# espresso3389/MioTTS-llama.cpp

Hardware: AMD Instinct MI355X
Metric: realtime factor (audio s / wall s) + stage ms llm/codec/istft, 1.7B Q4_K_M (higher is better)
Workload: dtype int8-dot (q4_K/q6_K x q8_K) + f32/f16 codec; 1 GPU; MioTTS-1.7B Q4_K_M single utterance, 700 speech tokens -> MioCodec -> iSTFT (28.0 s audio each) per GPU; model=MioTTS-1.7B Q4_K_M, global_batch=1, seq_len=700, parallelism=utterance-sharded x1 (no collective), devices_visible=1

## Files before the change

### miotts-llama.cpp_amd/csrc/hip/llm_attention.h

```cpp
#pragma once
#include "llm_device.h"

namespace mio {
namespace {

__device__ inline float load_resid(const float *x, int lo, int hi) {
    const int lane = threadIdx.x & 63;
    return lo + lane < hi ? x[lo + lane] : 0.0f;
}
__device__ inline float lane_value(float v, int i) {
    return __int_as_float(__builtin_amdgcn_readlane(__float_as_int(v), i));
}

template <int HD, int G, bool DG, bool WQ = false>
__device__ __forceinline__ bool attention_wg(const LlmDims &d, const float *q_norm, const float *k_norm,
                                             const float *bqkv, _Float16 *kc, _Float16 *vc, const LlmBuffers &b,
                                             int ch, int kvh, int pos, int *rdy) {
    constexpr bool kDiag = DG;
    using C = AttCfg<HD>;
    constexpr int PER = HD / 64;
    __shared__ float qs[G][HD];
    __shared__ float knew[HD], vnew[HD];
    using A = AttM<HD>;
    static_assert(C::NT == A::NT, "attention workgroup size");
// ... 61 lines not shown
    attend_chunk_mfma<HD, G>(qh, img, img + A::IMG, t0, pos, d.scale, b.part + head0 + (uint32_t)ch * C::REC, gs,
                             DG ? b.trace : nullptr);
    attn_merge_last<HD, G>(b.part, head0, gs, pos / ATT_CHUNK + 1, b.att_cnt + kvh, b.att + (size_t)kvh * G * HD, -1,
                           {}, 0, rdy, (kDiag && b.tl) ? MIO_TL_SLOT(b) : nullptr);
    return true;
}

template <int NP, int T, int SU, bool DG>
__device__ __forceinline__ void o_consumer(const LlmDims &d, const QMat &wo, const LlmBuffers &b, int ob, int no) {
    constexpr bool kDiag = DG;
    extern __shared__ __attribute__((aligned(16))) char smem[];
    const int K = wo.k;
    const Smem s = carve(smem, K);
    int lo, hi;
    wave_range(wo.rows, lo, hi, ob, no);
    const float xres = load_resid(b.x, lo, hi);
    Frag ga[Cfg<NP, SU>::U], gb[Cfg<NP, SU>::U];
    load_first<T, NP, 1, SU, MIO_SMALL_AUX>(wo, wo, lo, hi, ga, gb);
    if (MIO_TIDX == 0)
        wait_count(b.att_cnt + kRdyOff + kRdyStride * (blockIdx.x & (kRdyShards - 1)), d.n_kv, b.att_cnt + kRdyFlag);
    asm volatile("s_barrier" ::: "memory");
    MIO_TL_MARK(b, 3);
    XRegs<NP> xr;
    load_x<NP, 16>(b.att, nullptr, K, xr);
    x_after_weights(xr);
    MIO_TL_MARK1(b);
    plain_quant(xr, K, akind(T), s, MIO_TL_DIAGSLOT(b));
    MIO_TL_MARK(b, 2);
    stream_rows_lanes<T, NP, 1, SU, MIO_SMALL_AUX>(wo, wo, lo, hi, ga, gb, s.a, [&](int row, float v, float) {
        b.x[row] = v + xres;
    });
}

}
}
```

### miotts-llama.cpp_amd/csrc/hip/llm_device.h

```cpp
#pragma once

#include <cfloat>
#include <climits>
#include <cstdio>
#include <cstdlib>
#include <type_traits>

#include "llm_kernels.h"

#pragma clang fp contract(off)

#ifndef MIO_TIDX
#define MIO_TIDX threadIdx.x
#endif

namespace mio {
namespace {
constexpr bool kDiag = true;
#define MIO_TRACE(bufs, k)                                                                    \
    do {                                                                                      \
        if (kDiag && (bufs).trace && blockIdx.x == 0 && blockIdx.y == 0 && MIO_TIDX == 0) { \
            asm volatile("" ::: "memory");                                                    \
            (bufs).trace[k] = __builtin_readcyclecounter();                                   \
            if ((k) == 0 || (k) == 15) (bufs).trace[16 + (k)] = __builtin_amdgcn_s_memrealtime(); \
// ... 291 lines not shown
    float4 w[XV];
};

template <int XV>
__device__ __forceinline__ void x_after_weights(XRegs<XV> &xr) {
#pragma unroll
    for (int i = 0; i < XV; ++i)
        asm volatile("" : "+v"(xr.v[i].x), "+v"(xr.v[i].y), "+v"(xr.v[i].z), "+v"(xr.v[i].w), "+v"(xr.w[i].x),
                     "+v"(xr.w[i].y), "+v"(xr.w[i].z), "+v"(xr.w[i].w));
}

template <int XV, int XAUX = 0>
__device__ inline void load_x(const float *x, const float *w, int K, XRegs<XV> &xr) {
    const auto rx = __builtin_amdgcn_make_buffer_rsrc(const_cast<float *>(x), 0, x ? K * 4 : 0, 0x00020000);
    const auto rw = __builtin_amdgcn_make_buffer_rsrc(const_cast<float *>(w), 0, w ? K * 4 : 0, 0x00020000);
#pragma unroll
    for (int i = 0; i < XV; ++i) {
        const int e = (MIO_TIDX + i * MT) * 4;
        const u32x4 a = __builtin_amdgcn_raw_buffer_load_b128(rx, e * 4, 0, XAUX);
        const u32x4 c = __builtin_amdgcn_raw_buffer_load_b128(rw, e * 4, 0, 0);
        xr.v[i] = make_float4(__uint_as_float(a.x), __uint_as_float(a.y), __uint_as_float(a.z), __uint_as_float(a.w));
        xr.w[i] = make_float4(__uint_as_float(c.x), __uint_as_float(c.y), __uint_as_float(c.z), __uint_as_float(c.w));
    }
}

__host__ __device__ constexpr int akind(int T) { return T == 30 ? 2 : (T == 8 ? 0 : 1); }

__device__ __forceinline__ uint32_t f32_to_bf16(float f) {
    const uint32_t u = __float_as_uint(f);
    if ((u & 0x7fffffffu) > 0x7f800000u) return (u >> 16) | 64u;
    return (u + (0x7fffu + ((u >> 16) & 1u))) >> 16;
}

template <int XV>
__device__ __forceinline__ void quant_regs(const float4 (&v)[XV], int K, int ak, const ActL &a) {
    const int lane = MIO_TIDX & 63, wave = __builtin_amdgcn_readfirstlane(MIO_TIDX >> 6);
    if (ak == 1) {
        q8k_regs<XV>(v, K, a);
    } else if (ak == 2) {
#pragma unroll
        for (int j = 0; j < XV; ++j) {
            const int e = (MIO_TIDX + j * MT) * 4;
            if (e < K)
                *reinterpret_cast<uint2 *>(a.qs + 2 * e) =
                    make_uint2(f32_to_bf16(v[j].x) | (f32_to_bf16(v[j].y) << 16),
                               f32_to_bf16(v[j].z) | (f32_to_bf16(v[j].w) << 16));
// ... 275 lines not shown
        r.lo = *reinterpret_cast<const int4 *>(a.qs + e);
        r.hi = *reinterpret_cast<const int4 *>(a.qs + e2);
        r.b0 = a.bs[e >> 4];
        r.b1 = a.bs[e2 >> 4];
        r.d = a.d[sbc];
    } else if constexpr (T == 30) {
        auto at = [&](int i) {
            const int e = min(pass * 2048 + 512 * i + 8 * lane, K - 8);
            return *reinterpret_cast<const int4 *>(a.qs + 2 * e);
        };
        r.lo = at(0), r.hi = at(1), r.lo2 = at(2), r.hi2 = at(3);
        r.b0 = r.b1 = 0;
        r.d = 0.0f;
    } else {
        const int nb = K >> 5, b = pass * 64 + lane, bc = b < nb ? b : 0;
        r.lo = *reinterpret_cast<const int4 *>(a.qs + 32 * bc);
        r.hi = *reinterpret_cast<const int4 *>(a.qs + 32 * bc + 16);
        r.b0 = r.b1 = 0;
        r.d = a.d[bc];
    }
    return r;
}

template <int T>
__device__ __forceinline__ float dot_frag(const Frag &f, const ALane &al, int K, int pass) {
    const int lane = MIO_TIDX & 63;
    if constexpr (T == 12 || T == 13) {
        const int jj = (lane & 7) >> 1;
        uint4 h;
        auto bc = [&]<int CTRL>() {
            if constexpr (T == 12) return (uint32_t)dpp_perm<CTRL>((int)f.c);
            else return (uint32_t)dpp_i<CTRL>((int)f.c);
        };
        h.x = bc.template operator()<0x00>();
        h.y = bc.template operator()<0x55>();
        h.z = bc.template operator()<0xAA>();
        h.w = bc.template operator()<0xFF>();
        const uint32_t wlo = jj < 2 ? h.y : (jj == 2 ? h.z : h.w);
        const uint32_t whi = jj < 2 ? h.z : h.w;
        const uint32_t F = __builtin_amdgcn_alignbit(whi, wlo, (24 * jj) & 31);
        const int sc0 = F & 63, m0 = (F >> 6) & 63, sc1 = (F >> 12) & 63, m1 = (F >> 18) & 63;
        auto lo = [&](uint32_t q, uint32_t h) {
            if constexpr (T == 13) return (int)((q & M4) | (((h >> (2 * jj)) & 0x01010101u) << 4));
            else return (int)(q & M4);
        };
        auto hi = [&](uint32_t q, uint32_t h) {
            if constexpr (T == 13) return (int)(((q >> 4) & M4) | (((h >> (2 * jj + 1)) & 0x01010101u) << 4));
            else return (int)((q >> 4) & M4);
        };
        int dlo = 0, dhi = 0;
        dlo = sdot4(lo(f.a.x, f.b.x), al.lo.x, dlo);
        dlo = sdot4(lo(f.a.y, f.b.y), al.lo.y, dlo);
        dlo = sdot4(lo(f.a.z, f.b.z), al.lo.z, dlo);
        dlo = sdot4(lo(f.a.w, f.b.w), al.lo.w, dlo);
        dhi = sdot4(hi(f.a.x, f.b.x), al.hi.x, dhi);
        dhi = sdot4(hi(f.a.y, f.b.y), al.hi.y, dhi);
        dhi = sdot4(hi(f.a.z, f.b.z), al.hi.z, dhi);
        dhi = sdot4(hi(f.a.w, f.b.w), al.hi.w, dhi);
        int isum = __mul24(sc0, dlo) + __mul24(sc1, dhi);
        int imin = __mul24(m0, al.b0) + __mul24(m1, al.b1);
        isum = sum8_i(isum);
        imin = sum8_i(imin);
        const float d = h2f(h.x & 0xFFFF) * al.d;
        const float dmin = h2f(h.x >> 16) * al.d;
        float v = d * (float)isum;
        v = v - dmin * (float)imin;
        return pass * 8 + (lane >> 3) < (K >> 8) ? v : 0.0f;
    } else if constexpr (T == 14) {
        const int shl = 2 * ((lane & 3) >> 1);
        auto lo = [&](uint32_t l, uint32_t h) { return (int)((l & M4) | ((h << (4 - shl)) & 0x30303030u)); };
        auto hi = [&](uint32_t l, uint32_t h) { return (int)(((l >> 4) & M4) | ((h >> shl) & 0x30303030u)); };
        int dlo = 0, dhi = 0;
        dlo = sdot4(lo(f.a.x, f.b.x), al.lo.x, dlo);
        dlo = sdot4(lo(f.a.y, f.b.y), al.lo.y, dlo);
        dlo = sdot4(lo(f.a.z, f.b.z), al.lo.z, dlo);
        dlo = sdot4(lo(f.a.w, f.b.w), al.lo.w, dlo);
        dhi = sdot4(hi(f.a.x, f.b.x), al.hi.x, dhi);
        dhi = sdot4(hi(f.a.y, f.b.y), al.hi.y, dhi);
        dhi = sdot4(hi(f.a.z, f.b.z), al.hi.z, dhi);
        dhi = sdot4(hi(f.a.w, f.b.w), al.hi.w, dhi);
        const int sa = (int)(int8_t)(f.c & 0xFF), sb = (int)(int8_t)(f.c >> 8);
        int isum = __mul24(sa, dlo - 32 * al.b0) + __mul24(sb, dhi - 32 * al.b1);
        isum = sum8_i(isum);
        const float d = h2f(f.e) * al.d;
        const float v = d * (float)isum;
        return pass * 8 + (lane >> 3) < (K >> 8) ? v : 0.0f;
    } else if constexpr (T == 30) {
        typedef __bf16 bf2 __attribute__((ext_vector_type(2)));
        float acc = 0.0f;
        auto dot8 = [&](const uint4 &w, const int4 &x, int i) {
            const bool ok = pass * 2048 + 512 * i + 8 * lane < K;
            const uint4 ww = ok ? w : make_uint4(0, 0, 0, 0);
            const uint4 xx = ok ? make_uint4((uint32_t)x.x, (uint32_t)x.y, (uint32_t)x.z, (uint32_t)x.w)
                                : make_uint4(0, 0, 0, 0);
            acc = __builtin_amdgcn_fdot2_f32_bf16(__builtin_bit_cast(bf2, ww.x), __builtin_bit_cast(bf2, xx.x), acc, false);
            acc = __builtin_amdgcn_fdot2_f32_bf16(__builtin_bit_cast(bf2, ww.y), __builtin_bit_cast(bf2, xx.y), acc, false);
            acc = __builtin_amdgcn_fdot2_f32_bf16(__builtin_bit_cast(bf2, ww.z), __builtin_bit_cast(bf2, xx.z), acc, false);
            acc = __builtin_amdgcn_fdot2_f32_bf16(__builtin_bit_cast(bf2, ww.w), __builtin_bit_cast(bf2, xx.w), acc, false);
        };
        dot8(f.a, al.lo, 0);
        dot8(f.b, al.hi, 1);
        dot8(f.a2, al.lo2, 2);
        dot8(f.b2, al.hi2, 3);
        return acc;
    } else {
        int s = 0;
        s = sdot4((int)f.a.x, al.lo.x, s);
        s = sdot4((int)f.a.y, al.lo.y, s);
        s = sdot4((int)f.a.z, al.lo.z, s);
        s = sdot4((int)f.a.w, al.lo.w, s);
        s = sdot4((int)f.b.x, al.hi.x, s);
        s = sdot4((int)f.b.y, al.hi.y, s);
        s = sdot4((int)f.b.z, al.hi.z, s);
        s = sdot4((int)f.b.w, al.hi.w, s);
        const float v = (float)s * (h2f(f.e) * al.d);
        return pass * 64 + lane < (K >> 5) ? v : 0.0f;
    }
}

template <int T>
__device__ __forceinline__ float row_total(float acc) {
    if constexpr (T == 8 || T == 30) acc = sum8_f(acc);
    return sum_lanes7(acc);
}

template <int NP, int SU = 0>
struct Cfg {
    static constexpr int U = SU ? SU : (NP == 1 ? 4 : 3);
    static constexpr int NG = SU ? 1 : 2;
    static constexpr bool AREG = NP <= 3;
};

template <int T, int NP, int NM, int SU = 0, int AUX = MIO_WEIGHT_AUX>
__device__ __forceinline__ void load_group(const QMat W0, const QMat W1, int lo, int n, int u0,
                                           Frag (&f)[Cfg<NP, SU>::U], int split = INT_MAX) {
#pragma unroll
    for (int j = 0; j < Cfg<NP, SU>::U; ++j) {
        const int u = __builtin_amdgcn_readfirstlane(max(0, min(u0 + j, n - 1)));
        const int p = u % NP, m = (u / NP) % NM, i = u / (NP * NM);
        if constexpr (NM == 1) {
            const int r = __builtin_amdgcn_readfirstlane(lo + i);
            f[j] = load_frag<T, AUX>(r >= split ? W1 : W0, r >= split ? r - split : r, p);
        } else {
            f[j] = load_frag<T, AUX>(m ? W1 : W0, lo + i, p);
        }
    }
}

// ... 44 lines not shown
                }
            }
        }
    };
    for (int u0 = 0;;) {
        consume(A, u0);
        if (trace && u0 == 0 && blockIdx.x == 0 && MIO_TIDX == 0) trace[3] = __builtin_readcyclecounter();
        if constexpr (Cfg<NP, SU>::NG == 1) break;
        u0 += U;
        if (u0 >= n) break;
        load_group<T, NP, NM, SU, AUX>(W0, W1, lo, n, u0 + U, A, split);
        consume(B, u0);
        u0 += U;
        if (u0 >= n) break;
        load_group<T, NP, NM, SU, AUX>(W0, W1, lo, n, u0 + U, B, split);
    }
}

template <int T, int NP, int NM, int SU = 0, int AUX = MIO_WEIGHT_AUX, class Fin>
__device__ __forceinline__ void stream_rows_lanes(const QMat W0, const QMat W1, int lo, int hi,
                                                  Frag (&A)[Cfg<NP, SU>::U], Frag (&B)[Cfg<NP, SU>::U], const ActL &a,
                                                  Fin &&fin, int split = INT_MAX, unsigned long long *trace = nullptr) {
    const int lane = MIO_TIDX & 63;
    if constexpr (SU != 0 && SU / (NM * NP) == 1) {
        stream_rows<T, NP, NM, SU, AUX>(W0, W1, lo, hi, A, B, a, [&](int row, float v0, float v1) {
            if (lane == 0) fin(row, v0, v1);
        }, split, trace);
        return;
    }
    float p0 = 0.0f, p1 = 0.0f;
    stream_rows<T, NP, NM, SU, AUX>(W0, W1, lo, hi, A, B, a, [&](int row, float v0, float v1) {
        const int k = (row - lo) & 63;
        p0 = lane == k ? v0 : p0;
        if constexpr (NM == 2) p1 = lane == k ? v1 : p1;
        if constexpr (SU == 0) {
            if (k == 63) fin(row - 63 + lane, p0, p1);
        }
    }, split, trace);
    const int rest = SU == 0 ? (hi - lo) & 63 : hi - lo;
    if (lane < rest) fin(hi - rest + lane, p0, p1);
}

template <int T, int NP, int NM, int SU = 0, int AUX = MIO_WEIGHT_AUX>
__device__ __forceinline__ void load_first(const QMat W0, const QMat W1, int lo, int hi, Frag (&A)[Cfg<NP, SU>::U],
                                           Frag (&B)[Cfg<NP, SU>::U], int split = INT_MAX) {
    const int n = (hi - lo) * NM * NP;
// ... 614 lines not shown
```

### miotts-llama.cpp_amd/csrc/hip/llm_kernels.h

```cpp
#pragma once

#include <hip/hip_runtime.h>

#include <cstdint>

namespace mio {

#ifndef MIO_ATT_CHUNK
#define MIO_ATT_CHUNK 64
#endif
constexpr int kAttChunk = MIO_ATT_CHUNK;
constexpr int kTlSlots = 2048;
static_assert(kAttChunk == 32 || kAttChunk == 64 || kAttChunk == 128, "attention chunk");

struct QMat {
    int type;
    int rows, k;
    const uint8_t *p0, *p1, *p2, *p3;
};

inline QMat qmat_rows(const QMat &q, int r0, int n) {
    size_t rb[4] = {0, 0, 0, 0};
    switch (q.type) {
        case 8: rb[0] = (size_t)q.k, rb[1] = (size_t)q.k / 32 * 2; break;
// ... 161 lines not shown
    int g = rows / 8;
    g = g < n_wg ? g : n_wg;
    return g < 2 ? 2 : g;
}
int matvec_grid(const LlmDims &d, int rows);
bool att_o_supported(int hd, int G);
bool layer_att_supported(const LlmDims &d, const LayerW &L);
bool ffn_fused_supported(const LlmDims &d, const LayerW &L);
void launch_layer_att(const LlmDims &d, const LayerW &L, _Float16 *kc, _Float16 *vc, const LlmBuffers &b, bool dg,
                      hipStream_t s);
constexpr int kRdyOff = 64, kRdyShards = 8, kRdyStride = 64;
constexpr int kRdyFlag = kRdyOff + kRdyShards * kRdyStride;
constexpr int kQkvOff = kRdyFlag + 64, kQkvStride = 64, kQkvMax = 64;
constexpr int kFfnOff = kQkvOff + kQkvStride * kQkvMax, kFfnShards = 8, kFfnStride = 64;
constexpr int kFfnRdy = kFfnOff + kFfnShards * kFfnStride;
constexpr int kAttCntInts = kFfnRdy + kFfnShards * kFfnStride;
int pick_np(int K);
size_t matvec_lds(int K);
int max_wave_units(int rows, int grid, int np, int nm);
int pick_su(int units, int np);
void launch_attn_in(const LlmDims &d, const LayerW &L, int il, const QMat &tok_embd, const LlmBuffers &b, bool dg,
                    hipStream_t s);
void launch_debug_matvec(const QMat &W, const QMat *up, const float *x, float *y, int n_wg, hipStream_t s);
size_t debug_act_record_bytes(int K);
void launch_debug_act_quant(int type, const float *x, const float *w, int K, float eps, bool sc1, void *out,
                            hipStream_t s);
size_t debug_act_bytes(int K);
void launch_debug_mmq(const QMat &W, const QMat &up, int mode, const float *x, int nt, char *act, float *y,
                      hipStream_t s);

}
```

### miotts-llama.cpp_amd/csrc/hip/llm_kernels.hip

```cpp
#include "llm_attention.h"

#include <algorithm>
#include <cstdlib>

#pragma clang fp contract(off)

namespace mio {
namespace {



template <int NP, int T, int SU, bool DG>
__global__ __launch_bounds__(MT) void k_attn_out(LlmDims d, QMat wo, LlmBuffers b) {
    constexpr bool kDiag = DG;
    extern __shared__ __attribute__((aligned(16))) char smem[];
    MIO_TRACE(b, 0);
    MIO_TL_BEGIN(b);
    const int K = wo.k;
    const Smem s = carve(smem, K);
    int lo, hi;
    wave_range(d, wo.rows, lo, hi);
    const uint32_t dn = done_issue(b);
    XRegs<NP> xr;
    load_x(b.att, nullptr, K, xr);
    const float xres = load_resid(b.x, lo, hi);
    Frag ga[Cfg<NP, SU>::U], gb[Cfg<NP, SU>::U];
    load_first<T, NP, 1, SU, MIO_SMALL_AUX>(wo, wo, lo, hi, ga, gb);
    x_after_weights(xr);
    if (done_now(dn)) return;
    MIO_TRACE(b, 1);
    MIO_TL_MARK1(b);
    plain_quant(xr, K, akind(T), s, MIO_TL_DIAGSLOT(b));
    MIO_TRACE(b, 2);
    MIO_TL_MARK(b, 2);
    stream_rows_lanes<T, NP, 1, SU, MIO_SMALL_AUX>(wo, wo, lo, hi, ga, gb, s.a, [&](int row, float v, float) {
        b.x[row] = v + xres;
    });
    MIO_TL_END(b);
    MIO_TRACE(b, 15);
}

template <int NP, int T, int SU, bool DG>
__global__ __launch_bounds__(MT) void k_conv_out(LlmDims d, QMat wo, const float *conv_w, float *ring, LlmBuffers b) {
    constexpr bool kDiag = DG;
    extern __shared__ __attribute__((aligned(16))) char smem[];
    MIO_TRACE(b, 0);
    MIO_TL_BEGIN(b);
    const int K = wo.k;
    const Smem s = carve(smem, K);
    const uint32_t dn = done_issue(b);
    const int pos = cur_pos(b.st, d);
// ... 58 lines not shown
    MIO_TRACE(b, 1);
    MIO_TL_MARK1(b);
    rmsnorm_quant(xr, K, d.eps, akind(T), s, MIO_TL_DIAGSLOT(b));
    MIO_TRACE(b, 2);
    MIO_TL_MARK(b, 2);
    stream_rows_lanes<T, NP, 2, SU>(gate, up, lo, hi, ga, gb, s.a, [&](int row, float g, float u) {
        b.h[row] = silu_f(g) * u;
    }, INT_MAX, DG ? b.trace : nullptr);
    if (adv && blockIdx.x == 0 && MIO_TIDX == 0) advance_state(b.st, d);
    MIO_TL_END(b);
    MIO_TRACE(b, 15);
}

template <int NP, int T, int SU, bool DG>
__global__ __launch_bounds__(MT) void k_ffn_down(LlmDims d, QMat down, LlmBuffers b) {
    constexpr bool kDiag = DG;
    extern __shared__ __attribute__((aligned(16))) char smem[];
    MIO_TRACE(b, 0);
    MIO_TL_BEGIN(b);
    const int K = down.k;
    const Smem s = carve(smem, K);
    const uint32_t dn = done_issue(b);
    XRegs<NP> xr;
    load_x(b.h, nullptr, K, xr);
    int lo, hi;
    wave_range(d, down.rows, lo, hi);
    const float xres = load_resid(b.x, lo, hi);
    Frag ga[Cfg<NP, SU>::U], gb[Cfg<NP, SU>::U];
    load_first<T, NP, 1, SU>(down, down, lo, hi, ga, gb);
    x_after_weights(xr);
    if (done_now(dn)) return;
    MIO_TRACE(b, 1);
    MIO_TL_MARK1(b);
    plain_quant(xr, K, akind(T), s, MIO_TL_DIAGSLOT(b));
    MIO_TRACE(b, 2);
    MIO_TL_MARK(b, 2);
    stream_rows_lanes<T, NP, 1, SU>(down, down, lo, hi, ga, gb, s.a, [&](int row, float v, float) {
        b.x[row] = v + xres;
    }, INT_MAX, DG ? b.trace : nullptr);
    MIO_TL_END(b);
    MIO_TRACE(b, 15);
}

template <int NP, int T, int SU, int NPD, int TD, int SUD, bool DG>
__global__ __launch_bounds__(MT) void k_ffn(LlmDims d, const float *norm_w, QMat gate, QMat up, QMat down,
                                            LlmBuffers b, int adv, int GI) {
    constexpr bool kDiag = DG;
    extern __shared__ __attribute__((aligned(16))) char smem[];
    MIO_TRACE(b, 0);
    MIO_TL_BEGIN(b);
    const uint32_t dn = done_issue(b);
    if ((int)blockIdx.x < GI) {
        const int K = d.n_embd;
// ... 31 lines not shown
                last = __hip_atomic_fetch_add((__attribute__((address_space(1))) int *)(b.att_cnt + kFfnOff + kFfnStride * sh),
                                              1, __ATOMIC_RELAXED, __HIP_MEMORY_SCOPE_AGENT) == n_sh - 1;
            }
            if (__builtin_amdgcn_readfirstlane(last) && MIO_TIDX < kFfnShards)
                __hip_atomic_fetch_add((__attribute__((address_space(1))) int *)(b.att_cnt + kFfnRdy + kFfnStride * MIO_TIDX),
                                       1, __ATOMIC_RELAXED, __HIP_MEMORY_SCOPE_AGENT);
        }
    } else {
        const int K = down.k;
        const Smem s = carve(smem, K);
        const int GD = (int)gridDim.x - GI, ob = (int)blockIdx.x - GI;
        int lo, hi;
        wave_range(down.rows, lo, hi, ob, GD);
        const float xres = load_resid(b.x, lo, hi);
        Frag ga[Cfg<NPD, SUD>::U], gb[Cfg<NPD, SUD>::U];
        load_first<TD, NPD, 1, SUD>(down, down, lo, hi, ga, gb);
        if (done_now(dn)) return;
        if (MIO_TIDX == 0)
            wait_count(b.att_cnt + kFfnRdy + kFfnStride * (blockIdx.x & (kFfnShards - 1)), min(GI, kFfnShards),
                       b.att_cnt + kRdyFlag);
        asm volatile("s_barrier" ::: "memory");
        MIO_TL_MARK(b, 3);
        XRegs<NPD> xr;
        load_x<NPD, 16>(b.h, nullptr, K, xr);
        x_after_weights(xr);
        MIO_TL_MARK1(b);
        plain_quant(xr, K, akind(TD), s, MIO_TL_DIAGSLOT(b));
        MIO_TL_MARK(b, 2);
        stream_rows_lanes<TD, NPD, 1, SUD>(down, down, lo, hi, ga, gb, s.a, [&](int row, float v, float) {
            b.x[row] = v + xres;
        });
    }
    MIO_TL_END(b);
    MIO_TRACE(b, 15);
}

#define MIO_FFN_SHAPES(X) \
    X(1, 12, 6, 3, 12, 3)  \
    X(1, 12, 6, 3, 14, 3)  \
    X(1, 13, 6, 3, 13, 3)  \
    X(1, 13, 6, 3, 14, 3)  \
    X(1, 14, 6, 3, 14, 3)  \
    X(1, 30, 6, 3, 30, 3)  \
    X(1, 8, 2, 1, 8, 1)    \
    X(1, 8, 2, 1, 14, 1)   \
    X(1, 8, 0, 6, 8, 0)    \
    X(1, 14, 0, 6, 14, 0)

// ... 362 lines not shown
```

### miotts-llama.cpp_amd/csrc/testlib/debug_capi.cpp

```cpp
#include <cstring>
#include <vector>

#include "common.h"
#include "gguf.h"
#include "llm.h"
#include "llm_kernels.h"
#include "mio_hip_test.h"
#include "quant.h"

namespace {
int debug_matvec(mio_hip_device *d, uint32_t type, const void *gguf_rows, const void *gguf_up, int rows, int k,
                 const float *x, float *y) {
    MIO_REQUIRE(d && gguf_rows && x && y && rows > 0 && k > 0, MIO_ERR_INVALID, "debug_matvec: bad args");
    MIO_REQUIRE(type == mio::GGML_Q8_0 || type == mio::GGML_Q4_K || type == mio::GGML_Q5_K ||
                    type == mio::GGML_Q6_K || type == mio::GGML_BF16 || (!gguf_up && mio::repacks_to_q8_0(type)),
                MIO_ERR_UNSUPPORTED, "debug_matvec: type %u", type);
    const bool k32 = type == mio::GGML_Q8_0 || type == mio::GGML_BF16 || mio::repacks_to_q8_0(type);
    MIO_REQUIRE(k % (k32 ? 32 : 256) == 0, MIO_ERR_INVALID, "debug_matvec: k %d", k);
    int rc = mio::bind(d);
    if (rc) return rc;
    std::vector<uint8_t> q80;
    if (mio::repacks_to_q8_0(type)) {
        q80.resize((size_t)rows * (k / 32) * sizeof(mio::BlockQ8_0));
        mio::repack_to_q8_0(type, gguf_rows, rows, k, q80.data());
        gguf_rows = q80.data();
        type = mio::GGML_Q8_0;
    }
    const mio::SplitLayout L = mio::split_layout(type, rows, k);
    const int nm = gguf_up ? 2 : 1;
    std::vector<uint8_t> host(L.bytes * nm);
    mio::to_split(type, gguf_rows, rows, k, host.data());
    if (gguf_up) mio::to_split(type, gguf_up, rows, k, host.data() + L.bytes);
    uint8_t *dw = nullptr;
    float *dx = nullptr, *dy = nullptr;
    MIO_HIP_CHECK(hipMalloc(&dw, L.bytes * nm));
    MIO_HIP_CHECK(hipMalloc(&dx, (size_t)k * 4));
    MIO_HIP_CHECK(hipMalloc(&dy, (size_t)rows * 4));
    hipMemcpy(dw, host.data(), L.bytes * nm, hipMemcpyHostToDevice);
    hipMemcpy(dx, x, (size_t)k * 4, hipMemcpyHostToDevice);
    auto qm = [&](uint8_t *base) {
        return mio::QMat{(int)type, rows, k, base + L.off[0], base + L.off[1], base + L.off[2], base + L.off[3]};
    };
    const mio::QMat q = qm(dw), up = qm(dw + (gguf_up ? L.bytes : 0));
    mio::launch_debug_matvec(q, gguf_up ? &up : nullptr, dx, dy, d->n_cu > 0 ? d->n_cu : 256, d->stream);
    hipError_t e = hipStreamSynchronize(d->stream);
    if (e == hipSuccess) e = hipMemcpy(y, dy, (size_t)rows * 4, hipMemcpyDeviceToHost);
    hipFree(dw), hipFree(dx), hipFree(dy);
    MIO_HIP_CHECK(e);
    return MIO_OK;
}
}

extern "C" int mio_hip_debug_matvec(mio_hip_device *d, uint32_t type, const void *gguf_rows, int rows, int k,
                                    const float *x, float *y) {
    return debug_matvec(d, type, gguf_rows, nullptr, rows, k, x, y);
}

extern "C" int mio_hip_debug_matvec_swiglu(mio_hip_device *d, uint32_t type, const void *gguf_gate,
                                           const void *gguf_up, int rows, int k, const float *x, float *y) {
    MIO_REQUIRE(gguf_up, MIO_ERR_INVALID, "debug_matvec_swiglu: bad args");
    return debug_matvec(d, type, gguf_gate, gguf_up, rows, k, x, y);
}

extern "C" int mio_hip_debug_act_quant(mio_hip_device *d, uint32_t type, const float *x, const float *w, int k,
                                       float eps, int sc1, int8_t *qs, float *dd, int16_t *bs) {
    MIO_REQUIRE(d && x && qs && dd && bs && k > 0, MIO_ERR_INVALID, "debug_act_quant: bad args");
    MIO_REQUIRE(type == mio::GGML_Q8_0 || type == mio::GGML_Q4_K || type == mio::GGML_BF16, MIO_ERR_UNSUPPORTED,
                "debug_act_quant: type %u", type);
    MIO_REQUIRE(k % (type == mio::GGML_Q4_K ? 256 : 32) == 0 && k <= 12288, MIO_ERR_INVALID,
                "debug_act_quant: k %d", k);
    int rc = mio::bind(d);
    if (rc) return rc;
    const size_t nb = mio::debug_act_record_bytes(k);
    float *dx = nullptr, *dw = nullptr;
    char *dr = nullptr;
    MIO_HIP_CHECK(hipMalloc(&dx, (size_t)k * 4));
    MIO_HIP_CHECK(hipMalloc(&dw, (size_t)k * 4));
    MIO_HIP_CHECK(hipMalloc(&dr, nb));
    hipMemcpy(dx, x, (size_t)k * 4, hipMemcpyHostToDevice);
    if (w) hipMemcpy(dw, w, (size_t)k * 4, hipMemcpyHostToDevice);
    mio::launch_debug_act_quant((int)type, dx, w ? dw : nullptr, k, eps, sc1 != 0, dr, d->stream);
    hipError_t e = hipGetLastError();
    if (e == hipSuccess) e = hipStreamSynchronize(d->stream);
    std::vector<char> rec(nb);
// ... 94 lines not shown
```

### miotts-llama.cpp_amd/csrc/testlib/debug_kernels.hip

```cpp
#include "llm_device.h"

#pragma clang fp contract(off)

namespace mio {
namespace {
template <int NP, int T, int NM>
__global__ __launch_bounds__(MT) void k_debug_matvec(QMat W, QMat U, const float *x, float *y) {
    extern __shared__ __attribute__((aligned(16))) char smem[];
    const int K = W.k;
    const Smem s = carve(smem, K);
    XRegs<NP> xr;
    load_x(x, nullptr, K, xr);
    int lo, hi;
    wave_range(W.rows, lo, hi, blockIdx.x, gridDim.x);
    Frag ga[Cfg<NP>::U], gb[Cfg<NP>::U];
    load_first<T, NP, NM>(W, U, lo, hi, ga, gb);
    plain_quant(xr, K, akind(T), s);
    stream_rows_lanes<T, NP, NM>(W, U, lo, hi, ga, gb, s.a, [&](int row, float v, float u) {
        y[row] = NM == 2 ? silu_f(v) * u : v;
    });
}

template <int NP, int T, int XAUX>
__global__ __launch_bounds__(MT) void k_debug_act_quant(const float *x, const float *w, int K, float eps,
                                                        uint32_t *out) {
    extern __shared__ __attribute__((aligned(16))) char smem[];
    const Smem s = carve(smem, K);
    XRegs<NP> xr;
    load_x<NP, XAUX>(x, w, K, xr);
    if (w)
        rmsnorm_quant(xr, K, eps, akind(T), s);
    else
        plain_quant(xr, K, akind(T), s);
    const int n = (int)((smem_bytes(K) - 128) / 4);
    for (int i = MIO_TIDX; i < n; i += MT) out[i] = reinterpret_cast<const uint32_t *>(smem)[i];
}
}

size_t debug_act_record_bytes(int K) { return smem_bytes(K) - 128; }

void launch_debug_act_quant(int type, const float *x, const float *w, int K, float eps, bool sc1, void *out,
// ... 1 lines not shown
    dispatch_nt(K, type, [&]<int NP, int T>() {
        if (sc1)
            hipLaunchKernelGGL((k_debug_act_quant<NP, T, 16>), dim3(1), dim3(MT), matvec_lds(K), s, x, w, K, eps,
                               (uint32_t *)out);
        else
            hipLaunchKernelGGL((k_debug_act_quant<NP, T, 0>), dim3(1), dim3(MT), matvec_lds(K), s, x, w, K, eps,
                               (uint32_t *)out);
    });
}

void launch_debug_matvec(const QMat &W, const QMat *up, const float *x, float *y, int n_wg, hipStream_t s) {
    LlmDims d{};
    d.n_wg = n_wg;
    dispatch_nt(W.k, W.type, [&]<int NP, int T>() {
        if (up)
            hipLaunchKernelGGL((k_debug_matvec<NP, T, 2>), dim3(matvec_grid(d, W.rows)), dim3(MT), matvec_lds(W.k), s,
                               W, *up, x, y);
        else
            hipLaunchKernelGGL((k_debug_matvec<NP, T, 1>), dim3(matvec_grid(d, W.rows)), dim3(MT), matvec_lds(W.k), s,
                               W, W, x, y);
    });
}

}
```

### miotts-llama.cpp_amd/python/miotts_amd/__init__.py

```python
from __future__ import annotations

import ctypes
import os
from typing import Optional

import numpy as np

PKG_ROOT = os.path.dirname(os.path.dirname(os.path.dirname(os.path.abspath(__file__))))
REPO_ROOT = os.path.dirname(PKG_ROOT)
BUILD_DIR = os.environ.get("MIO_BUILD_DIR") or os.path.join(PKG_ROOT, "build")
LIB_PATH = os.path.join(BUILD_DIR, "libmiotts.so")
TEST_LIB_PATH = os.path.join(BUILD_DIR, "libmiotts_test.so")
INCLUDE_DIR = os.path.join(REPO_ROOT, "include")

MIO_IN_DEVICE = 1
MIO_OUT_DEVICE = 2
MIO_CODEC_INCREMENTAL = 4

_lib = None

_f32p = ctypes.POINTER(ctypes.c_float)
_i32p = ctypes.POINTER(ctypes.c_int32)
_vp = ctypes.c_void_p

# ... 96 lines not shown
        "mio_tokenize": (c_int, [_vp, ctypes.c_char_p, c_int, c_int, _vp, c_int, ctypes.POINTER(c_int)]),
        "mio_token_piece": (c_int, [_vp, ctypes.c_int32, ctypes.c_char_p, c_int, ctypes.POINTER(c_int)]),
        "mio_hip_llm_timeline": (c_int, [_vp, _vp, c_int, ctypes.POINTER(c_int)]),
        "mio_hip_codec_last_timings": (c_int, [_vp, _f32p]),
        "mio_hip_codec_last_reused": (c_int, [_vp, ctypes.POINTER(c_int)]),
        "mio_hip_codec_last_flops": (c_int, [_vp, ctypes.POINTER(ctypes.c_double)]),
        "mio_hip_llm_load_ms": (c_int, [_vp, ctypes.POINTER(ctypes.c_double)]),
        "mio_hip_llm_steps_issued": (c_int, [_vp, ctypes.POINTER(c_int)]),
        "mio_hip_llm_tail": (c_int, [_vp, ctypes.POINTER(c_int), ctypes.POINTER(c_int), ctypes.POINTER(ctypes.c_float)]),
        "mio_hip_llm_step_kinds": (c_int, [_vp, _vp, c_int, ctypes.POINTER(c_int)]),
        "mio_hip_llm_batch_step_launches": (c_int, [_vp, c_int, ctypes.POINTER(c_int)]),
        "mio_hip_llm_conv_ring": (c_int, [_vp, c_int, _vp, c_int]),
        "mio_hip_llm_eval_layers": (c_int, [_vp, ctypes.c_int32, c_int, _vp, _vp]),
        "mio_hip_llm_kv_rows": (c_int, [_vp, c_int, c_int, _vp, _vp]),
        "mio_hip_llm_set_kv_rows": (c_int, [_vp, c_int, c_int, c_int, _vp, _vp]),
        "mio_hip_llm_debug_attention": (c_int, [_vp, c_int, c_int, c_int, _vp, _vp]),
        "mio_hip_llm_set_sampling": (c_int, [_vp, ctypes.POINTER(Sampling)]),
        "mio_hip_llm_get_sampling": (c_int, [_vp, ctypes.POINTER(Sampling)]),
        "mio_hip_llm_debug_sample_chain": (c_int, [_vp, _vp, _vp, c_int, ctypes.POINTER(Sampling), ctypes.c_float,
                                                   ctypes.c_uint64, c_int, ctypes.c_int32, ctypes.c_int32, _i32p,
                                                   _i32p, _i32p, _vp]),
        "mio_hip_debug_matvec": (c_int, [_vp, ctypes.c_uint32, _vp, c_int, c_int, _vp, _vp]),
        "mio_hip_debug_matvec_swiglu": (c_int, [_vp, ctypes.c_uint32, _vp, _vp, c_int, c_int, _vp, _vp]),
        "mio_hip_debug_act_quant": (c_int, [_vp, ctypes.c_uint32, _vp, _vp, c_int, ctypes.c_float, c_int, _vp, _vp,
                                            _vp]),
        "mio_quantize_rows": (c_int, [ctypes.c_uint32, _vp, c_int, c_int, _vp]),
        "mio_dequantize_rows": (c_int, [ctypes.c_uint32, _vp, c_int, c_int, _vp]),
        "mio_hip_debug_mmq": (c_int, [_vp, ctypes.c_uint32, _vp, c_int, c_int, _vp, c_int, c_int, _vp, _vp]),
        "mio_hip_debug_codec_gemm": (c_int, [_vp, _vp, _vp, _vp, _vp, _vp, _vp, _vp, ctypes.POINTER(c_int)]),
        "mio_hip_debug_codec_conv": (c_int, [_vp, _vp, c_int, c_int, c_int, c_int, _vp, c_int, _vp, c_int, _vp, _vp,
                                             ctypes.POINTER(c_int)]),
        "mio_hip_debug_codec_rownorm": (c_int, [_vp, _vp, c_int, c_int, ctypes.c_float, c_int, _vp, _vp, c_int, _vp,
                                                ctypes.POINTER(c_int)]),
        "mio_hip_debug_codec_groupnorm": (c_int, [_vp, _vp, c_int, c_int, c_int, ctypes.c_float, _vp, _vp, _vp,
                                                  ctypes.POINTER(c_int)]),
        "mio_hip_debug_codec_band_attention": (c_int, [_vp, _vp, c_int, c_int, c_int, _vp, _vp,
                                                       ctypes.POINTER(c_int)]),
        "mio_hip_debug_codec_cond_gemv": (c_int, [_vp, _vp, _vp, _vp, c_int, c_int, c_int, _vp,
                                                  ctypes.POINTER(c_int)]),
        "mio_hip_debug_codec_embed": (c_int, [_vp, _vp, c_int, c_int, _vp, c_int, _vp, ctypes.POINTER(c_int)]),
        "mio_hip_llm_info": (c_int, [_vp, _i32p]),
        "mio_hip_llm_weight_bytes": (c_int, [_vp, ctypes.POINTER(ctypes.c_uint64)]),
        "mio_hip_llm_eval": (c_int, [_vp, ctypes.c_int32, c_int, _vp]),
        "mio_hip_llm_prefill": (c_int, [_vp, _vp, c_int, _vp]),
        "mio_hip_llm_logits": (c_int, [_vp, _vp]),
        "mio_hip_llm_generate": (c_int, [_vp, _vp, c_int, c_int, ctypes.c_float, ctypes.c_uint64,
# ... 493 lines not shown
    out = np.empty((rows_bytes.shape[0], k), np.float32)
    check(lib().mio_dequantize_rows(qtype, _ptr(rows_bytes), rows_bytes.shape[0], k, _ptr(out)))
    return out


def debug_matvec(dev: Device, qtype: int, w_rows: np.ndarray, k: int, x: np.ndarray) -> np.ndarray:
    w_rows = np.ascontiguousarray(w_rows)
    x = np.ascontiguousarray(x, dtype=np.float32)
    y = np.empty(w_rows.shape[0], np.float32)
    check(lib().mio_hip_debug_matvec(dev.h, qtype, _ptr(w_rows), w_rows.shape[0], k, _ptr(x), _ptr(y)))
    return y


def debug_matvec_swiglu(dev: Device, qtype: int, gate_rows: np.ndarray, up_rows: np.ndarray, k: int,
                        x: np.ndarray) -> np.ndarray:
    gate_rows, up_rows = np.ascontiguousarray(gate_rows), np.ascontiguousarray(up_rows)
    x = np.ascontiguousarray(x, dtype=np.float32)
    y = np.empty(gate_rows.shape[0], np.float32)
    check(lib().mio_hip_debug_matvec_swiglu(dev.h, qtype, _ptr(gate_rows), _ptr(up_rows), gate_rows.shape[0], k,
                                            _ptr(x), _ptr(y)))
    return y


def debug_act_quant(dev: Device, qtype: int, x: np.ndarray, w: Optional[np.ndarray] = None, eps: float = 1e-6,
                    sc1: bool = False):
    x = np.ascontiguousarray(x, dtype=np.float32)
    k = x.shape[0]
    wv = np.ascontiguousarray(w, dtype=np.float32) if w is not None else None
    qs, d, bs = np.empty(2 * k, np.int8), np.empty(k // 32 + 8, np.float32), np.empty(k // 16 + 8, np.int16)
    check(lib().mio_hip_debug_act_quant(dev.h, qtype, _ptr(x), _ptr(wv) if wv is not None else None, k, eps,
                                        int(sc1), _ptr(qs), _ptr(d), _ptr(bs)))
    return qs, d, bs


def debug_mmq(dev: Device, qtype: int, w_rows: np.ndarray, k: int, x: np.ndarray, mode: int = 0,
              y_in: Optional[np.ndarray] = None, up_rows: Optional[np.ndarray] = None) -> np.ndarray:
    w_rows = np.ascontiguousarray(w_rows)
    x = np.ascontiguousarray(x, dtype=np.float32)
    y = np.zeros((x.shape[0], w_rows.shape[0]), np.float32) if y_in is None else np.array(y_in, np.float32)
    up = np.ascontiguousarray(up_rows) if up_rows is not None else None
    check(lib().mio_hip_debug_mmq(dev.h, qtype, _ptr(w_rows), w_rows.shape[0], k, _ptr(x), x.shape[0], mode,
                                  _ptr(up) if up is not None else None, _ptr(y)))
    return y


SENTINEL_F32 = 0x7FC5A5A5
# ... 174 lines not shown
```

Before: 58.85 x realtime (audio s / wall s).

## Reduce paired matvec rows jointly with cross-lane swaps and drop unused weight loads

Adds a joint-row reduction path for Q4_K/Q6_K single-pass matvecs with small row counts per wave. Two rows' partial dot sums are reduced together using DPP and permlane16/32 swaps instead of separate full-wave reductions per row. It also adds a plain x loader that skips the always-null norm-weight buffer load and its register pinning in the o-projection and down-projection consumers. A debug group-matvec entry point is added for testing. The joint path adds complex lane bookkeeping for which lane holds each row's result, which is a correctness risk.

New measurement: 60.08 x realtime (audio s / wall s), median of 6. 1.02x the previous value.

```diff
diff --git a/miotts-llama.cpp_amd/csrc/hip/llm_attention.h b/miotts-llama.cpp_amd/csrc/hip/llm_attention.h
--- a/miotts-llama.cpp_amd/csrc/hip/llm_attention.h
+++ b/miotts-llama.cpp_amd/csrc/hip/llm_attention.h
@@ -107,8 +107,8 @@
     asm volatile("s_barrier" ::: "memory");
     MIO_TL_MARK(b, 3);
     XRegs<NP> xr;
-    load_x<NP, 16>(b.att, nullptr, K, xr);
-    x_after_weights(xr);
+    load_x_plain<NP, 16>(b.att, K, xr);
+    x_after_weights_plain(xr);
     MIO_TL_MARK1(b);
     plain_quant(xr, K, akind(T), s, MIO_TL_DIAGSLOT(b));
     MIO_TL_MARK(b, 2);
diff --git a/miotts-llama.cpp_amd/csrc/hip/llm_device.h b/miotts-llama.cpp_amd/csrc/hip/llm_device.h
--- a/miotts-llama.cpp_amd/csrc/hip/llm_device.h
+++ b/miotts-llama.cpp_amd/csrc/hip/llm_device.h
@@ -337,6 +337,22 @@
         xr.v[i] = make_float4(__uint_as_float(a.x), __uint_as_float(a.y), __uint_as_float(a.z), __uint_as_float(a.w));
         xr.w[i] = make_float4(__uint_as_float(c.x), __uint_as_float(c.y), __uint_as_float(c.z), __uint_as_float(c.w));
     }
+}
+
+template <int XV, int XAUX = 0>
+__device__ inline void load_x_plain(const float *x, int K, XRegs<XV> &xr) {
+    const auto rx = __builtin_amdgcn_make_buffer_rsrc(const_cast<float *>(x), 0, x ? K * 4 : 0, 0x00020000);
+#pragma unroll
+    for (int i = 0; i < XV; ++i) {
+        const int e = (MIO_TIDX + i * MT) * 4;
+        const u32x4 a = __builtin_amdgcn_raw_buffer_load_b128(rx, e * 4, 0, XAUX);
+        xr.v[i] = make_float4(__uint_as_float(a.x), __uint_as_float(a.y), __uint_as_float(a.z), __uint_as_float(a.w));
+    }
+}
+template <int XV>
+__device__ __forceinline__ void x_after_weights_plain(XRegs<XV> &xr) {
+#pragma unroll
+    for (int i = 0; i < XV; ++i) asm volatile("" : "+v"(xr.v[i].x), "+v"(xr.v[i].y), "+v"(xr.v[i].z), "+v"(xr.v[i].w));
 }
 
 __host__ __device__ constexpr int akind(int T) { return T == 30 ? 2 : (T == 8 ? 0 : 1); }
@@ -658,9 +674,15 @@
     return r;
 }
 
+struct LaneTerms {
+    int isum, imin;
+    uint32_t hd;
+};
 template <int T>
-__device__ __forceinline__ float dot_frag(const Frag &f, const ALane &al, int K, int pass) {
+__device__ __forceinline__ LaneTerms lane_terms(const Frag &f, const ALane &al) {
+    static_assert(T == 12 || T == 13 || T == 14, "K-quants");
     const int lane = MIO_TIDX & 63;
+    LaneTerms t;
     if constexpr (T == 12 || T == 13) {
         const int jj = (lane & 7) >> 1;
         uint4 h;
@@ -693,16 +715,10 @@
         dhi = sdot4(hi(f.a.y, f.b.y), al.hi.y, dhi);
         dhi = sdot4(hi(f.a.z, f.b.z), al.hi.z, dhi);
         dhi = sdot4(hi(f.a.w, f.b.w), al.hi.w, dhi);
-        int isum = __mul24(sc0, dlo) + __mul24(sc1, dhi);
-        int imin = __mul24(m0, al.b0) + __mul24(m1, al.b1);
-        isum = sum8_i(isum);
-        imin = sum8_i(imin);
-        const float d = h2f(h.x & 0xFFFF) * al.d;
-        const float dmin = h2f(h.x >> 16) * al.d;
-        float v = d * (float)isum;
-        v = v - dmin * (float)imin;
-        return pass * 8 + (lane >> 3) < (K >> 8) ? v : 0.0f;
-    } else if constexpr (T == 14) {
+        t.isum = __mul24(sc0, dlo) + __mul24(sc1, dhi);
+        t.imin = __mul24(m0, al.b0) + __mul24(m1, al.b1);
+        t.hd = h.x;
+    } else {
         const int shl = 2 * ((lane & 3) >> 1);
         auto lo = [&](uint32_t l, uint32_t h) { return (int)((l & M4) | ((h << (4 - shl)) & 0x30303030u)); };
         auto hi = [&](uint32_t l, uint32_t h) { return (int)(((l >> 4) & M4) | ((h >> shl) & 0x30303030u)); };
@@ -716,10 +732,35 @@
         dhi = sdot4(hi(f.a.z, f.b.z), al.hi.z, dhi);
         dhi = sdot4(hi(f.a.w, f.b.w), al.hi.w, dhi);
         const int sa = (int)(int8_t)(f.c & 0xFF), sb = (int)(int8_t)(f.c >> 8);
-        int isum = __mul24(sa, dlo - 32 * al.b0) + __mul24(sb, dhi - 32 * al.b1);
-        isum = sum8_i(isum);
-        const float d = h2f(f.e) * al.d;
-        const float v = d * (float)isum;
+        t.isum = __mul24(sa, dlo - 32 * al.b0) + __mul24(sb, dhi - 32 * al.b1);
+        t.imin = 0;
+        t.hd = f.e;
+    }
+    return t;
+}
+
+template <int T>
+__device__ __forceinline__ float sb_term(int isum, int imin, uint32_t hd, float ad) {
+    if constexpr (T == 14) {
+        const float d = h2f(hd) * ad;
+        return d * (float)isum;
+    } else {
+        const float d = h2f(hd & 0xFFFF) * ad;
+        const float dmin = h2f(hd >> 16) * ad;
+        float v = d * (float)isum;
+        v = v - dmin * (float)imin;
+        return v;
+    }
+}
+
+template <int T>
+__device__ __forceinline__ float dot_frag(const Frag &f, const ALane &al, int K, int pass) {
+    const int lane = MIO_TIDX & 63;
+    if constexpr (T == 12 || T == 13 || T == 14) {
+        const LaneTerms t = lane_terms<T>(f, al);
+        const int isum = sum8_i(t.isum);
+        const int imin = T == 14 ? 0 : sum8_i(t.imin);
+        const float v = sb_term<T>(isum, imin, t.hd, al.d);
         return pass * 8 + (lane >> 3) < (K >> 8) ? v : 0.0f;
     } else if constexpr (T == 30) {
         typedef __bf16 bf2 __attribute__((ext_vector_type(2)));
@@ -760,6 +801,81 @@
     return sum_lanes7(acc);
 }
 
+__device__ __forceinline__ int pair_sum8(int a, int b, bool side_b) {
+    a += dpp_perm<0x141>(a);
+    b += dpp_perm<0x141>(b);
+    int r = side_b ? b : a;
+    r += dpp_perm<0xB1>(r);
+    r += dpp_perm<0x4E>(r);
+    return r;
+}
+template <int T>
+__device__ __forceinline__ float pair_term(const Frag &fa, const Frag &fb, const ALane &al, bool side_b, bool in_k) {
+    const LaneTerms a = lane_terms<T>(fa, al), b = lane_terms<T>(fb, al);
+    const int isum = pair_sum8(a.isum, b.isum, side_b);
+    const int imin = T == 14 ? 0 : pair_sum8(a.imin, b.imin, side_b);
+    const float v = sb_term<T>(isum, imin, side_b ? b.hd : a.hd, al.d);
+    return in_k ? v : 0.0f;
+}
+__device__ __forceinline__ float ror8_add(float v) {
+    return v + __int_as_float(dpp_perm<0x128>(__float_as_int(v)));
+}
+__device__ __forceinline__ float swapadd16(float a, float b) {
+    const auto r = __builtin_amdgcn_permlane16_swap(__float_as_uint(a), __float_as_uint(b), false, false);
+    return __uint_as_float(r[1]) + __uint_as_float(r[0]);
+}
+__device__ __forceinline__ float swapadd32(float a, float b) {
+    const auto r = __builtin_amdgcn_permlane32_swap(__float_as_uint(a), __float_as_uint(b), false, false);
+    return __uint_as_float(r[1]) + __uint_as_float(r[0]);
+}
+template <int T, int NP, int NM, int SU>
+constexpr bool joint_rows = (T == 12 || T == 14) && NP == 1 && SU >= 2 && (NM == 2 || SU <= 4);
+
+template <int T, int NM, int SU, class Fin>
+__device__ __forceinline__ void rows_joint(const Frag (&F)[SU], const ActL &a, int K, int lo, int hi, Fin &&fin) {
+    constexpr int NPR = (SU + 1) / 2;
+    static_assert(NM == 1 || NPR <= 4, "one 16-lane row per row pair");
+    static_assert(NM == 2 || SU <= 8, "a row's parking lane and its pair side");
+    const int lane = MIO_TIDX & 63;
+    const ALane al = load_alane<T>(a, K, 0);
+    const bool side_b = (lane & 4) != 0, in_k = (lane >> 3) < (K >> 8);
+    float x[NPR];
+#pragma unroll
+    for (int p = 0; p < NPR; ++p) {
+        float acc = 0.0f;
+        acc += pair_term<T>(F[2 * p], F[2 * p + 1 < SU ? 2 * p + 1 : 2 * p], al, side_b, in_k);
+        x[p] = ror8_add(acc);
+    }
+    if constexpr (NM == 2) {
+        float r;
+        if constexpr (NPR == 1) {
+            const float q = swapadd16(x[0], x[0]);
+            r = swapadd32(q, q);
+        } else if constexpr (NPR == 2) {
+            const float q = swapadd16(x[0], x[1]);
+            r = swapadd32(q, q);
+        } else {
+            const float q = swapadd16(x[0], x[1]), q2 = swapadd16(x[2], x[NPR - 1]);
+            r = swapadd32(q, q2);
+        }
+        const float r1 = dpp_f<0x104>(r);
+        if ((lane & 15) == 0 && (lane >> 4) < hi - lo) fin(lo + (lane >> 4), r, r1);
+    } else {
+        float p0 = 0.0f;
+#pragma unroll
+        for (int p = 0; p < NPR; ++p) {
+            const float q = swapadd16(x[p], x[p]);
+            const float r = swapadd32(q, q), rs = dpp_f<0x104>(r);
+#pragma unroll
+            for (int u = 2 * p; u < 2 * p + 2 && u < SU; ++u) {
+                const float v = ((u >> 2) & 1) == (u & 1) ? r : rs;
+                p0 = u == 0 ? v : (lane == u ? v : p0);
+            }
+        }
+        if (lane < hi - lo) fin(lo + lane, p0, 0.0f);
+    }
+}
+
 template <int NP, int SU = 0>
 struct Cfg {
     static constexpr int U = SU ? SU : (NP == 1 ? 4 : 3);
@@ -850,6 +966,12 @@
                                                   Frag (&A)[Cfg<NP, SU>::U], Frag (&B)[Cfg<NP, SU>::U], const ActL &a,
                                                   Fin &&fin, int split = INT_MAX, unsigned long long *trace = nullptr) {
     const int lane = MIO_TIDX & 63;
+    if constexpr (joint_rows<T, NP, NM, SU>) {
+        if (hi <= lo) return;
+        rows_joint<T, NM, SU>(A, a, W0.k, lo, hi, fin);
+        if (trace && blockIdx.x == 0 && MIO_TIDX == 0) trace[3] = __builtin_readcyclecounter();
+        return;
+    }
     if constexpr (SU != 0 && SU / (NM * NP) == 1) {
         stream_rows<T, NP, NM, SU, AUX>(W0, W1, lo, hi, A, B, a, [&](int row, float v0, float v1) {
             if (lane == 0) fin(row, v0, v1);
diff --git a/miotts-llama.cpp_amd/csrc/hip/llm_kernels.h b/miotts-llama.cpp_amd/csrc/hip/llm_kernels.h
--- a/miotts-llama.cpp_amd/csrc/hip/llm_kernels.h
+++ b/miotts-llama.cpp_amd/csrc/hip/llm_kernels.h
@@ -207,6 +207,8 @@
 void launch_attn_in(const LlmDims &d, const LayerW &L, int il, const QMat &tok_embd, const LlmBuffers &b, bool dg,
                     hipStream_t s);
 void launch_debug_matvec(const QMat &W, const QMat *up, const float *x, float *y, int n_wg, hipStream_t s);
+bool launch_debug_matvec_group(const QMat &W, const QMat *up, const float *x, float *y, int su, int grid,
+                               hipStream_t s);
 size_t debug_act_record_bytes(int K);
 void launch_debug_act_quant(int type, const float *x, const float *w, int K, float eps, bool sc1, void *out,
                             hipStream_t s);
diff --git a/miotts-llama.cpp_amd/csrc/hip/llm_kernels.hip b/miotts-llama.cpp_amd/csrc/hip/llm_kernels.hip
--- a/miotts-llama.cpp_amd/csrc/hip/llm_kernels.hip
+++ b/miotts-llama.cpp_amd/csrc/hip/llm_kernels.hip
@@ -22,11 +22,11 @@
     wave_range(d, wo.rows, lo, hi);
     const uint32_t dn = done_issue(b);
     XRegs<NP> xr;
-    load_x(b.att, nullptr, K, xr);
+    load_x_plain(b.att, K, xr);
     const float xres = load_resid(b.x, lo, hi);
     Frag ga[Cfg<NP, SU>::U], gb[Cfg<NP, SU>::U];
     load_first<T, NP, 1, SU, MIO_SMALL_AUX>(wo, wo, lo, hi, ga, gb);
-    x_after_weights(xr);
+    x_after_weights_plain(xr);
     if (done_now(dn)) return;
     MIO_TRACE(b, 1);
     MIO_TL_MARK1(b);
@@ -131,13 +131,13 @@
     const Smem s = carve(smem, K);
     const uint32_t dn = done_issue(b);
     XRegs<NP> xr;
-    load_x(b.h, nullptr, K, xr);
+    load_x_plain(b.h, K, xr);
     int lo, hi;
     wave_range(d, down.rows, lo, hi);
     const float xres = load_resid(b.x, lo, hi);
     Frag ga[Cfg<NP, SU>::U], gb[Cfg<NP, SU>::U];
     load_first<T, NP, 1, SU>(down, down, lo, hi, ga, gb);
-    x_after_weights(xr);
+    x_after_weights_plain(xr);
     if (done_now(dn)) return;
     MIO_TRACE(b, 1);
     MIO_TL_MARK1(b);
@@ -215,8 +215,8 @@
         asm volatile("s_barrier" ::: "memory");
         MIO_TL_MARK(b, 3);
         XRegs<NPD> xr;
-        load_x<NPD, 16>(b.h, nullptr, K, xr);
-        x_after_weights(xr);
+        load_x_plain<NPD, 16>(b.h, K, xr);
+        x_after_weights_plain(xr);
         MIO_TL_MARK1(b);
         plain_quant(xr, K, akind(TD), s, MIO_TL_DIAGSLOT(b));
         MIO_TL_MARK(b, 2);
diff --git a/miotts-llama.cpp_amd/csrc/testlib/debug_capi.cpp b/miotts-llama.cpp_amd/csrc/testlib/debug_capi.cpp
--- a/miotts-llama.cpp_amd/csrc/testlib/debug_capi.cpp
+++ b/miotts-llama.cpp_amd/csrc/testlib/debug_capi.cpp
@@ -10,7 +10,7 @@
 
 namespace {
 int debug_matvec(mio_hip_device *d, uint32_t type, const void *gguf_rows, const void *gguf_up, int rows, int k,
-                 const float *x, float *y) {
+                 const float *x, float *y, int su = 0, int grid = 0) {
     MIO_REQUIRE(d && gguf_rows && x && y && rows > 0 && k > 0, MIO_ERR_INVALID, "debug_matvec: bad args");
     MIO_REQUIRE(type == mio::GGML_Q8_0 || type == mio::GGML_Q4_K || type == mio::GGML_Q5_K ||
                     type == mio::GGML_Q6_K || type == mio::GGML_BF16 || (!gguf_up && mio::repacks_to_q8_0(type)),
@@ -42,7 +42,15 @@
         return mio::QMat{(int)type, rows, k, base + L.off[0], base + L.off[1], base + L.off[2], base + L.off[3]};
     };
     const mio::QMat q = qm(dw), up = qm(dw + (gguf_up ? L.bytes : 0));
-    mio::launch_debug_matvec(q, gguf_up ? &up : nullptr, dx, dy, d->n_cu > 0 ? d->n_cu : 256, d->stream);
+    bool launched = true;
+    if (su > 0)
+        launched = mio::launch_debug_matvec_group(q, gguf_up ? &up : nullptr, dx, dy, su, grid, d->stream);
+    else
+        mio::launch_debug_matvec(q, gguf_up ? &up : nullptr, dx, dy, d->n_cu > 0 ? d->n_cu : 256, d->stream);
+    if (!launched) {
+        hipFree(dw), hipFree(dx), hipFree(dy);
+        MIO_REQUIRE(false, MIO_ERR_INVALID, "debug_matvec_group: su %d / grid %d for %d rows, k %d", su, grid, rows, k);
+    }
     hipError_t e = hipStreamSynchronize(d->stream);
     if (e == hipSuccess) e = hipMemcpy(y, dy, (size_t)rows * 4, hipMemcpyDeviceToHost);
     hipFree(dw), hipFree(dx), hipFree(dy);
@@ -60,6 +68,16 @@
                                            const void *gguf_up, int rows, int k, const float *x, float *y) {
     MIO_REQUIRE(gguf_up, MIO_ERR_INVALID, "debug_matvec_swiglu: bad args");
     return debug_matvec(d, type, gguf_gate, gguf_up, rows, k, x, y);
+}
+
+extern "C" int mio_hip_debug_matvec_group(mio_hip_device *d, uint32_t type, const void *gguf_gate,
+                                          const void *gguf_up, int rows, int k, int su, int grid, const float *x,
+                                          float *y) {
+    MIO_REQUIRE(su > 0 && grid > 0 && grid <= 4096, MIO_ERR_INVALID, "debug_matvec_group: su %d / grid %d", su, grid);
+    MIO_REQUIRE(type == mio::GGML_Q8_0 || type == mio::GGML_Q4_K || type == mio::GGML_Q5_K ||
+                    type == mio::GGML_Q6_K || type == mio::GGML_BF16,
+                MIO_ERR_UNSUPPORTED, "debug_matvec_group: type %u", type);
+    return debug_matvec(d, type, gguf_gate, gguf_up, rows, k, x, y, su, grid);
 }
 
 extern "C" int mio_hip_debug_act_quant(mio_hip_device *d, uint32_t type, const float *x, const float *w, int k,
diff --git a/miotts-llama.cpp_amd/csrc/testlib/debug_kernels.hip b/miotts-llama.cpp_amd/csrc/testlib/debug_kernels.hip
--- a/miotts-llama.cpp_amd/csrc/testlib/debug_kernels.hip
+++ b/miotts-llama.cpp_amd/csrc/testlib/debug_kernels.hip
@@ -17,6 +17,23 @@
     load_first<T, NP, NM>(W, U, lo, hi, ga, gb);
     plain_quant(xr, K, akind(T), s);
     stream_rows_lanes<T, NP, NM>(W, U, lo, hi, ga, gb, s.a, [&](int row, float v, float u) {
+        y[row] = NM == 2 ? silu_f(v) * u : v;
+    });
+}
+
+template <int NP, int T, int NM, int SU>
+__global__ __launch_bounds__(MT) void k_debug_matvec_group(QMat W, QMat U, const float *x, float *y) {
+    extern __shared__ __attribute__((aligned(16))) char smem[];
+    const int K = W.k;
+    const Smem s = carve(smem, K);
+    XRegs<NP> xr;
+    load_x(x, nullptr, K, xr);
+    int lo, hi;
+    wave_range(W.rows, lo, hi, blockIdx.x, gridDim.x);
+    Frag ga[Cfg<NP, SU>::U], gb[Cfg<NP, SU>::U];
+    load_first<T, NP, NM, SU>(W, U, lo, hi, ga, gb);
+    plain_quant(xr, K, akind(T), s);
+    stream_rows_lanes<T, NP, NM, SU>(W, U, lo, hi, ga, gb, s.a, [&](int row, float v, float u) {
         y[row] = NM == 2 ? silu_f(v) * u : v;
     });
 }
@@ -64,4 +81,35 @@
     });
 }
 
+bool launch_debug_matvec_group(const QMat &W, const QMat *up, const float *x, float *y, int su, int grid,
+                               hipStream_t s) {
+    const int np = pick_np(W.k), nm = up ? 2 : 1;
+    if (grid < 1 || np > 3) return false;
+    for (int b = 0; b < grid; ++b) {
+        const int ra = (int)((long long)W.rows * b / grid), rb = (int)((long long)W.rows * (b + 1) / grid);
+        for (int w = 0; w < MW; ++w)
+            if (((rb - ra) * (w + 1) / MW - (rb - ra) * w / MW) * np * nm > su) return false;
+    }
+    bool ok = false;
+    dispatch_nt(W.k, W.type, [&]<int NP, int T>() {
+        auto go = [&]<int NM, int SU>() {
+            hipLaunchKernelGGL((k_debug_matvec_group<NP, T, NM, SU>), dim3(grid), dim3(MT), matvec_lds(W.k), s, W,
+                               up ? *up : W, x, y);
+            ok = true;
+        };
+        if constexpr (NP == 1) {
+            if (nm == 1 && su == 2) go.template operator()<1, 2>();
+            if (nm == 1 && su == 3) go.template operator()<1, 3>();
+            if (nm == 1 && su == 4) go.template operator()<1, 4>();
+            if (nm == 1 && su == 6) go.template operator()<1, 6>();
+            if (nm == 2 && su == 2) go.template operator()<2, 2>();
+            if (nm == 2 && su == 4) go.template operator()<2, 4>();
+            if (nm == 2 && su == 6) go.template operator()<2, 6>();
+        } else if constexpr (NP == 3) {
+            if (nm == 1 && su == 3) go.template operator()<1, 3>();
+        }
+    });
+    return ok;
 }
+
+}
diff --git a/miotts-llama.cpp_amd/python/miotts_amd/__init__.py b/miotts-llama.cpp_amd/python/miotts_amd/__init__.py
--- a/miotts-llama.cpp_amd/python/miotts_amd/__init__.py
+++ b/miotts-llama.cpp_amd/python/miotts_amd/__init__.py
@@ -142,6 +142,7 @@
                                                    _i32p, _i32p, _vp]),
         "mio_hip_debug_matvec": (c_int, [_vp, ctypes.c_uint32, _vp, c_int, c_int, _vp, _vp]),
         "mio_hip_debug_matvec_swiglu": (c_int, [_vp, ctypes.c_uint32, _vp, _vp, c_int, c_int, _vp, _vp]),
+        "mio_hip_debug_matvec_group": (c_int, [_vp, ctypes.c_uint32, _vp, _vp, c_int, c_int, c_int, c_int, _vp, _vp]),
         "mio_hip_debug_act_quant": (c_int, [_vp, ctypes.c_uint32, _vp, _vp, c_int, ctypes.c_float, c_int, _vp, _vp,
                                             _vp]),
         "mio_quantize_rows": (c_int, [ctypes.c_uint32, _vp, c_int, c_int, _vp]),
@@ -681,6 +682,17 @@
     return y
 
 
+def debug_matvec_group(dev: Device, qtype: int, gate_rows: np.ndarray, up_rows: Optional[np.ndarray], k: int,
+                       x: np.ndarray, su: int, grid: int) -> np.ndarray:
+    gate_rows = np.ascontiguousarray(gate_rows)
+    up = np.ascontiguousarray(up_rows) if up_rows is not None else None
+    x = np.ascontiguousarray(x, dtype=np.float32)
+    y = np.empty(gate_rows.shape[0], np.float32)
+    check(lib().mio_hip_debug_matvec_group(dev.h, qtype, _ptr(gate_rows), _ptr(up) if up is not None else None,
+                                           gate_rows.shape[0], k, su, grid, _ptr(x), _ptr(y)))
+    return y
+
+
 def debug_act_quant(dev: Device, qtype: int, x: np.ndarray, w: Optional[np.ndarray] = None, eps: float = 1e-6,
                     sc1: bool = False):
     x = np.ascontiguousarray(x, dtype=np.float32)
```
